# ioloizou/g1_locomotion

Hardware: AMD Instinct MI355X
Metric: QP solves/sec, SRBD N=10 12-state/12-input (higher is better)
Workload: dtype f64; 1 GPU; configs[1]: batch=4096/GPU random SRBD states, N=10, 2-contact alternating single support friction cone, fp64; tails deferred (SRBDQP_FLAG_DEFER_TAIL: the ~4 % of a batch that reach a rho-restart mark finish in the next launch on their stream; srbdqp_flush inside the timed region, every batch complete when the clock stops); steps rotate over 4 distinct device batches; horizon=10, batch_per_gpu=4096, kernel=wave_defer_f64_n10_s2, streams=2, longest_first_hint=False, deferred_tails=True, world_size=1, distinct_batches=4, max_iter=250, rho_restart_iter=0, rho_restart_count=0, set_up_dtype=f64

## Files before the change

### g1_locomotion_amd/csrc/srbdqp_common.hpp

```cpp
#pragma once
#include <cstddef>
#include <hip/hip_runtime.h>
#include <stdint.h>

namespace srbdqp {

constexpr int kThreads = 256;
constexpr double kInf = 1.0e30;

struct KArgs {
    const double* x0;
    const double* xref;
    const double* foot;
    const double* pcom;
    const double* warm_u;
    const double* warm_y;
    const uint8_t* contact;
    double* u_out;
    double* x_out;
    double* y_out;
    int32_t* status;
    int32_t* iters;
    double* P_out;
    double* q_out;
    double* l_out;
    double* ub_out;
    const int32_t* perm;
    int defer_x0;
    int tile_sel;
    const int32_t* row_off;
    long long* stamps;
    double* ws;
    const double* rho_qp;
    double* rho_out;
    const float* resid_in;
    float* resid_out;
    const int32_t* count_ptr;
    int32_t* cap_list;
    int32_t* cap_count;
    int32_t iters_base;
    int32_t restart_every;
    int32_t restart_max;
    int32_t inline_in;
    int32_t y_capped_only;
    int32_t qp_span;
    double* u_dev;
    char* tail_lists;
    int32_t* tail_cnt;
    int32_t tail_cap, tail_wgs, tail_iin, tail_iout, tail_izero;
    int32_t done_cs;
    int32_t* done_flag;
    int32_t* done_count;
    int32_t done_value;
    int32_t B;
    int32_t mode;
    int32_t max_iter, check_every;
    double dt, inv_mass, iinv[3], mu, fzmin_s, fzmax_s, s;
    double sqrtq[12];
    double rs2;
    double rho, rho_eq, sigma, alpha, eps_abs, eps_rel;
    double rho_fz;
};

template <int N>
struct StagedIn {
    double x0[13];
    double xref[13 * N];
    double foot[12 * N];
    double pcom[3 * N];
    uint8_t contact[4 * N];
    uint8_t pad[(8 - (4 * N) % 8) % 8];
};
template <int N>
__device__ __forceinline__ const char* staged_in_base(const KArgs& a) {
    static_assert(sizeof(KArgs) % 8 == 0, "StagedIn follows KArgs without padding");
    if constexpr (sizeof(KArgs) + sizeof(StagedIn<N>) > 4096) return nullptr;
    else return a.inline_in ? (const char*)__builtin_amdgcn_kernarg_segment_ptr() + sizeof(KArgs) : nullptr;
}

struct QpIo {
    const double *x0, *xref, *foot, *pcom;
    const uint8_t* contact;
    double *u_out, *x_out, *y_out;
    int32_t *status, *iters;
};
__device__ __forceinline__ QpIo io_of(const KArgs& a) { return QpIo{a.x0, a.xref, a.foot, a.pcom, a.contact, a.u_out, a.x_out, a.y_out, a.status, a.iters}; }
struct TailRecHead {
    int32_t b, pass, done, pad;
    double rho;
    QpIo io;
};
static_assert(sizeof(TailRecHead) <= 16 * sizeof(double), "the header of a tail record is 16 doubles");
constexpr int kTailRecDoubles = 16 + 3 * 64;
constexpr int kStatusPending = 0;

#define SRBDQP_QP_INDEX(a) ((a).perm ? (a).perm[blockIdx.x] : (int)blockIdx.x)

__device__ __forceinline__ double restart_rho_of(double rho0, const float* r) {
    const double num = (double)r[0] / fmax((double)r[1], 1e-30), den = (double)r[2] / fmax((double)r[3], 1e-30);
    double r1 = rho0;
    if (num > 0.0 && den > 0.0 && num <= 1.0e30 && den <= 1.0e30) r1 = fmin(fmax(rho0 * sqrt(num / den), rho0 * 0.1), rho0 * 5.0);
    return r1;
}
#define SRBDQP_RESTART_SKIP(a, b) ((a).resid_in && (a).status[(b)] != 2)
__device__ __forceinline__ double rho_of_qp(const KArgs& a, int b) {
    const double r0 = a.rho_qp ? a.rho_qp[b] : a.rho;
    const double r = a.resid_in ? restart_rho_of(r0, a.resid_in + (size_t)b * 4) : r0;
    if (a.rho_out && threadIdx.x == 0) a.rho_out[b] = r;
    return r;
}
#define SRBDQP_RHO_OF(a, b) rho_of_qp((a), (b))

__device__ __forceinline__ float uni(float v) { return __int_as_float(__builtin_amdgcn_readfirstlane(__float_as_int(v))); }
__device__ __forceinline__ double uni(double v) {
    const int lo = __builtin_amdgcn_readfirstlane(__double2loint(v)), hi = __builtin_amdgcn_readfirstlane(__double2hiint(v));
    return __hiloint2double(hi, lo);
}

__device__ __forceinline__ double unis(double v) {
    int lo, hi;
    asm volatile("s_nop 1\n\tv_readfirstlane_b32 %0, %2\n\tv_readfirstlane_b32 %1, %3" : "=s"(lo), "=s"(hi) : "v"(__double2loint(v)), "v"(__double2hiint(v)));
    return __hiloint2double(hi, lo);
}

constexpr int kAbStride = 18;
template <int N>
__device__ __forceinline__ void de_tables(const double* CP, const double* T1, const double* T2, const double* SQ, const double dt2, double* DE, const int t, const int nthreads, const int nl = N) {
    for (int it = t; it < 9 * N; it += nthreads) {
        const int m = it / 9, k = it - 9 * m, p = k / 3, q = k - 3 * p;
        const double* Cm = CP + 9 * m;
        const double* t1 = T1 + 9 * m;
        const double d4 = dt2 * dt2;
        const double e0 = SQ[0] * SQ[0] * t1[q], e1 = SQ[1] * SQ[1] * t1[3 + q], e2 = SQ[2] * SQ[2] * t1[6 + q];
        double v = T2[9 * m + k] + Cm[p] * e0 + Cm[3 + p] * e1 + Cm[6 + p] * e2;
        v *= d4;
        v += (p == q) ? (double)(nl - m) * dt2 * SQ[6 + p] * SQ[6 + p] : 0.0;
        DE[18 * m + k] = v;
        DE[18 * m + 9 + k] = d4 * ((p == 0) ? e0 : (p == 1) ? e1 : e2);
    }
}
template <int N>
__device__ __forceinline__ void kasm_rows(const double* Jb, const double* CP, const double* DE, const double* SQ, const uint8_t* act, const int n_eff, const double s,
                                          const double dt2m, const double dtm, double* AB, const int t, const int nthreads, const int nrows) {
    const double s2 = s * s, dt4m2 = dt2m * dt2m, dt2m2 = dtm * dtm;
    for (int r = t; r < nrows; r += nthreads) {
        const bool on = r < n_eff;
        const int rr = on ? r : 0;
        const int e = rr / 3, x = rr - 3 * e, gc = act[e], j = gc >> 2;
        const double* Jp = Jb + j * 36 + 3 * (gc & 3) + x;
        const double J0 = Jp[0], J1 = Jp[12], J2 = Jp[24];
        const double* C = CP + 9 * j;
        const double* D = DE + 18 * j;
        double v[16];
        v[0] = J0; v[1] = J1; v[2] = J2;
#pragma unroll
        for (int l = 0; l < 3; ++l) v[3 + l] = -(C[3 * l] * J0 + C[3 * l + 1] * J1 + C[3 * l + 2] * J2);
        v[6] = 1.0; v[7] = -(double)j;
#pragma unroll
        for (int l = 0; l < 6; ++l) v[8 + l] = s2 * (D[3 * l] * J0 + D[3 * l + 1] * J1 + D[3 * l + 2] * J2);
        const int Ls = N - j;
        const double al = (double)(((Ls - 1) * Ls * (2 * Ls - 1)) / 6), be = (double)(((Ls - 1) * Ls) / 2);
        const double fa = SQ[3 + x] * SQ[3 + x] * dt4m2, fb = SQ[9 + x] * SQ[9 + x] * dt2m2;
        v[14] = s2 * (fa * (al + (double)j * be) + fb * (double)Ls);
        v[15] = s2 * fa * be;
        typedef double d2 __attribute__((ext_vector_type(2)));
        d2* row = reinterpret_cast<d2*>(AB + kAbStride * r);
#pragma unroll
        for (int i = 0; i < 8; ++i) row[i] = on ? (d2){v[2 * i], v[2 * i + 1]} : (d2){0.0, 0.0};
    }
}

__device__ __forceinline__ void kasm_tile(const double* AB, const int ta, const int tb, const int mcol, const int kq, const int n_eff, const double dgxy, const double dgz,
                                          double (&out)[4]) {
    typedef double d2 __attribute__((ext_vector_type(2)));
    const int c = 16 * tb + mcol;
    double Bv[8];
    {
        const d2* row = reinterpret_cast<const d2*>(AB + kAbStride * c + 8);
#pragma unroll
        for (int i = 0; i < 4; ++i) { const d2 v = row[i]; Bv[2 * i] = v[0]; Bv[2 * i + 1] = v[1]; }
    }
    const int cm3 = c - 3 * ((c * 0xAAAB) >> 17);
    const double dcol = (c < n_eff) ? ((cm3 < 2) ? dgxy : dgz) : 1.0;
#pragma unroll
    for (int q = 0; q < 4; ++q) {
        const int r = 16 * ta + kq + 4 * q;
        const d2* row = reinterpret_cast<const d2*>(AB + kAbStride * r);
        double Av[8];
#pragma unroll
        for (int i = 0; i < 4; ++i) { const d2 v = row[i]; Av[2 * i] = v[0]; Av[2 * i + 1] = v[1]; }
        double v = Av[0] * Bv[0];
#pragma unroll
        for (int i = 1; i < 6; ++i) v = fma(Av[i], Bv[i], v);
        const double ft = fma(Av[7], Bv[7], Av[6] * Bv[6]);
        const int d = r + 3 * 1024 - c, dm3 = d - 3 * ((d * 0xAAAB) >> 17);
        v += (dm3 == 0) ? ft : 0.0;
        v += (r == c) ? dcol : 0.0;
        out[q] = v;
    }
}

template <int N>
__device__ __forceinline__ double gx_row(const double* CP, const double* TF, const int i, const int kk, const double dt, const double dt2, const double dtm, const double dt2m) {
    double acc = 0.0;
    if (kk < 3) {
        const double* Ci = CP + i * 9 + kk * 3;
        const double c0 = Ci[0], c1 = Ci[1], c2 = Ci[2];
#pragma unroll 4
        for (int j = 0; j < N; ++j) {
            const double* Cj = CP + j * 9 + kk * 3;
            const double* tau = TF + 6 * j;
            const double term = (c0 - Cj[0]) * tau[0] + (c1 - Cj[1]) * tau[1] + (c2 - Cj[2]) * tau[2];
            acc += (j <= i) ? term : 0.0;
        }
        return acc * dt2;
    } else if (kk < 6) {
#pragma unroll 4
        for (int j = 0; j < N; ++j) { const double v = TF[6 * j + kk]; acc += (j <= i) ? (double)(i - j) * v : 0.0; }
        return acc * dt2m;
    } else {
#pragma unroll 4
        for (int j = 0; j < N; ++j) { const double v = TF[6 * j + kk - 6]; acc += (j <= i) ? v : 0.0; }
        return acc * ((kk < 9) ? dt : dtm);
    }
}

constexpr int kFirstCheck = 0;

#define SRBDQP_STAMP(a, b, idx) do { if ((a).stamps && threadIdx.x == 0) (a).stamps[(size_t)(b) * 16 + (idx)] = (long long)__builtin_amdgcn_s_memtime(); } while (0)

__device__ __forceinline__ void signal_done(const KArgs& a) {
    if (!a.done_flag) return;
    __threadfence_system();
    __syncthreads();
    if (threadIdx.x == 0) {
        bool last = true;
        if (a.B > 1) {
            last = (atomicAdd(a.done_count, 1) == a.B - 1);
            if (last) *a.done_count = 0;
        }
        if (last) __hip_atomic_store(a.done_flag, a.done_value, __ATOMIC_RELAXED, __HIP_MEMORY_SCOPE_SYSTEM);
    }
}

__device__ __forceinline__ unsigned long long done_cs_pack(int status, int iters) { return (unsigned long long)(unsigned)status | ((unsigned long long)(unsigned)iters << 32); }
__device__ __forceinline__ unsigned dpp_xor_row(unsigned v) {
    v ^= (unsigned)__builtin_amdgcn_update_dpp((int)v, (int)v, 0xB1, 0xF, 0xF, false);
    v ^= (unsigned)__builtin_amdgcn_update_dpp((int)v, (int)v, 0x4E, 0xF, 0xF, false);
    v ^= (unsigned)__builtin_amdgcn_update_dpp((int)v, (int)v, 0x141, 0xF, 0xF, false);
    v ^= (unsigned)__builtin_amdgcn_update_dpp((int)v, (int)v, 0x140, 0xF, 0xF, false);
    return v;
}
template <int BT>
__device__ __forceinline__ void signal_done_checksum(int32_t* done_flag, int32_t done_value, unsigned long long cs) {
    static_assert(BT % 16 == 0 && BT / 16 <= 16, "one 16-byte record per row of 16 lanes in 256 bytes");
    const unsigned lo = dpp_xor_row((unsigned)cs), hi = dpp_xor_row((unsigned)(cs >> 32));
    if ((threadIdx.x & 15) == 0) {
        uint4 v;
        v.x = (unsigned)done_value; v.y = (unsigned)(BT / 16); v.z = lo; v.w = hi;
        reinterpret_cast<uint4*>(done_flag)[threadIdx.x >> 4] = v;
    }
}

template <int N>
struct Dims {
    static constexpr int n = 12 * N;
    static constexpr int m = 20 * N;
    static constexpr int gtot = 72 * N * (N + 1);
    static constexpr int ME = (m + kThreads - 1) / kThreads;
    static constexpr int VE = (n + kThreads - 1) / kThreads;
};

template <int N, class L>
__device__ void load_and_linearise(const KArgs& a, int b, double* sm) {
    using S = L;
    const int t = threadIdx.x;
    const char* kin_ = staged_in_base<N>(a);
    const double* gx0 = kin_ ? reinterpret_cast<const double*>(kin_ + offsetof(StagedIn<N>, x0)) : a.x0 + (size_t)b * 13;
    const double* gxr = kin_ ? reinterpret_cast<const double*>(kin_ + offsetof(StagedIn<N>, xref)) : a.xref + (size_t)b * N * 13;
    const double* gft = kin_ ? reinterpret_cast<const double*>(kin_ + offsetof(StagedIn<N>, foot)) : a.foot + (size_t)b * N * 12;
    const uint8_t* gct = kin_ ? reinterpret_cast<const uint8_t*>(kin_ + offsetof(StagedIn<N>, contact)) : a.contact + (size_t)b * N * 4;
    uint8_t* sct = reinterpret_cast<uint8_t*>(sm + S::o_ct);
    constexpr int RX = (N * 13 + kThreads - 1) / kThreads, RF = (N * 12 + kThreads - 1) / kThreads;
    static_assert(N * 4 <= kThreads, "one thread per contact flag");
    const double* gpc = a.pcom ? (kin_ ? reinterpret_cast<const double*>(kin_ + offsetof(StagedIn<N>, pcom)) : a.pcom + (size_t)b * N * 3) : gx0;
    const double v_x0 = gx0[t < 13 ? t : 0];
    const uint8_t v_ct = gct[t < N * 4 ? t : 0];
    const double v_pc = gpc[(a.pcom && t < N * 3) ? t : 0];
    double v_xr[RX], v_ft[RF];
#pragma unroll
    for (int r = 0; r < RX; ++r) { const int i = t + r * kThreads; v_xr[r] = gxr[i < N * 13 ? i : 0]; }
#pragma unroll
    for (int r = 0; r < RF; ++r) { const int i = t + r * kThreads; v_ft[r] = gft[i < N * 12 ? i : 0]; }
    if (t < 13) sm[S::o_x0 + t] = v_x0;
    if (t >= 32 && t < 44) sm[S::o_sq + t - 32] = a.sqrtq[t - 32];
#pragma unroll
    for (int r = 0; r < RX; ++r) { const int i = t + r * kThreads; if (i < N * 13) sm[S::o_xref + i] = v_xr[r]; }
#pragma unroll
    for (int r = 0; r < RF; ++r) { const int i = t + r * kThreads; if (i < N * 12) sm[S::o_foot + i] = v_ft[r]; }
    if (t < N * 4) sct[t] = v_ct ? 1 : 0;
    if (a.pcom && t < N * 3) sm[S::o_pcom + t] = v_pc;
    __syncthreads();
    if (!a.pcom && t < N * 3) sm[S::o_pcom + t] = sm[S::o_xref + (t / 3) * 13 + 3 + (t % 3)];
    if (t < N) {
        double sn, cs;
        sincos(sm[S::o_xref + t * 13 + 2], &sn, &cs);
        double* T = sm + S::o_tm + t * 9;
        T[0] = cs;  T[1] = sn;  T[2] = 0.0;
        T[3] = -sn; T[4] = cs;  T[5] = 0.0;
        T[6] = 0.0; T[7] = 0.0; T[8] = 1.0;
    }
    __syncthreads();
    if (t < 9) {
        double acc = 0.0;
        for (int k = 0; k < N; ++k) { acc += sm[S::o_tm + k * 9 + t]; sm[S::o_cp + k * 9 + t] = acc; }
    }
    if (t < N * 12) {
        const int k = t / 12, cc = t % 12, ci = cc / 3, ax = cc % 3;
        const double cs = sm[S::o_tm + k * 9 + 0], sn = sm[S::o_tm + k * 9 + 1];
        const double i0 = a.iinv[0], i1 = a.iinv[1], i2 = a.iinv[2];
        const double w00 = cs * cs * i0 + sn * sn * i1, w01 = cs * sn * (i0 - i1), w11 = sn * sn * i0 + cs * cs * i1;
        const double rx = sm[S::o_foot + k * 12 + 3 * ci + 0] - sm[S::o_pcom + k * 3 + 0];
        const double ry = sm[S::o_foot + k * 12 + 3 * ci + 1] - sm[S::o_pcom + k * 3 + 1];
        const double rz = sm[S::o_foot + k * 12 + 3 * ci + 2] - sm[S::o_pcom + k * 3 + 2];
        const double s0 = (ax == 0) ? 0.0 : ((ax == 1) ? -rz : ry);
        const double s1 = (ax == 0) ? rz : ((ax == 1) ? 0.0 : -rx);
        const double s2 = (ax == 0) ? -ry : ((ax == 1) ? rx : 0.0);
        double* J = sm + S::o_J + k * 36;
        J[0 * 12 + cc] = w00 * s0 + w01 * s1;
        J[1 * 12 + cc] = w01 * s0 + w11 * s1;
        J[2 * 12 + cc] = i2 * s2;
    }
    __syncthreads();
}

template <int N, class L>
__device__ __forceinline__ double free_response(const KArgs& a, const double* sm, int i, int kk) {
    using S = L;
    const double* x0 = sm + S::o_x0;
    if (kk < 3) {
        const double* C = sm + S::o_cp + i * 9 + kk * 3;
        return x0[kk] + a.dt * (C[0] * x0[6] + C[1] * x0[7] + C[2] * x0[8]);
    } else if (kk < 6) {
        double v = x0[kk] + (double)(i + 1) * a.dt * x0[kk + 6];
        if (kk == 5) v += a.dt * a.dt * x0[12] * (double)((i * (i + 1)) / 2);
        return v;
    } else if (kk < 9) {
        return x0[kk];
    } else {
        double v = x0[kk];
        if (kk == 11) v += (double)(i + 1) * a.dt * x0[12];
        return v;
    }
}

template <int N, class L>
__device__ __forceinline__ void eh_entry(const KArgs& a, double* sm, const double* SQ, const int k) {
    const int i = k / 12, kk = k - 12 * i;
    sm[L::o_eh + k] = SQ[kk] * (free_response<N, L>(a, sm, i, kk) - sm[L::o_xref + i * 13 + kk]);
}

template <int N, class L>
__device__ __forceinline__ double free_response_sel(const KArgs& a, const double* sm, int i, int kk) {
    const double* x0 = sm + L::o_x0;
    const double* C = sm + L::o_cp + i * 9 + (kk < 3 ? kk : 0) * 3;
    const double xk = x0[kk];
    const double vr = xk + a.dt * (C[0] * x0[6] + C[1] * x0[7] + C[2] * x0[8]);
    const double vp = xk + (double)(i + 1) * a.dt * x0[(kk >= 3 && kk < 6) ? kk + 6 : 6];
    const double vz = vp + a.dt * a.dt * x0[12] * (double)((i * (i + 1)) / 2);
    const double vw = xk + (double)(i + 1) * a.dt * x0[12];
    return (kk < 3) ? vr : (kk < 5) ? vp : (kk == 5) ? vz : (kk == 11) ? vw : xk;
}

template <int N>
__device__ __forceinline__ void de_step(const double (&Cm)[9], const double (&t1)[9], const double (&t2)[9], const double* SQ, const double dt2, const int m, double* de) {
    const double d4 = dt2 * dt2;
#pragma unroll
    for (int k = 0; k < 9; ++k) {
        const int p = k / 3, q = k - 3 * p;
        const double e0 = SQ[0] * SQ[0] * t1[q], e1 = SQ[1] * SQ[1] * t1[3 + q], e2 = SQ[2] * SQ[2] * t1[6 + q];
        double v = t2[k] + Cm[p] * e0 + Cm[3 + p] * e1 + Cm[6 + p] * e2;
        v *= d4;
        if (p == q) v += (double)(N - m) * dt2 * SQ[6 + p] * SQ[6 + p];
        de[k] = v;
        de[9 + k] = d4 * ((p == 0) ? e0 : (p == 1) ? e1 : e2);
    }
}

__device__ __forceinline__ double lane_bcast(double v, int l) {
    const int lo = __builtin_amdgcn_readlane(__double2loint(v), l), hi = __builtin_amdgcn_readlane(__double2hiint(v), l);
    return __hiloint2double(hi, lo);
}

template <int NV>
__device__ __forceinline__ void block_max(double (&v)[NV], double* red) {
    const int lane = threadIdx.x & 63, wave = threadIdx.x >> 6;
#pragma unroll
    for (int q = 0; q < NV; ++q) {
        double x = v[q];
#pragma unroll
        for (int off = 32; off >= 1; off >>= 1) x = fmax(x, __shfl_xor(x, off));
        if (lane == 0) red[wave * 8 + q] = x;
    }
    __syncthreads();
#pragma unroll
    for (int q = 0; q < NV; ++q) v[q] = fmax(fmax(red[q], red[8 + q]), fmax(red[16 + q], red[24 + q]));
    __syncthreads();
}

template <int N, class L, int BT = kThreads, bool CS = false>
__device__ void rollout_and_store_to(const KArgs& a, double* u_out, double* x_out, int b, double* sm, const double* uh, double* scratch , unsigned long long* cs = nullptr) {
    using S = L;
    constexpr int n = Dims<N>::n;
    const int t = threadIdx.x;
    for (int c = t; c < n; c += BT) {
        const double v = a.s * uh[c];
        u_out[(size_t)b * n + c] = v;
        if constexpr (CS) *cs ^= (unsigned long long)__double_as_longlong(v);
    }
    if (a.u_dev) for (int c = t; c < n; c += BT) a.u_dev[(size_t)b * n + c] = a.s * uh[c];
    if (!x_out) return;
    const double* x0 = sm + S::o_x0;
    double* sj = scratch + 6 * N;
    for (int idx = t; idx < 6 * N; idx += BT) {
        const int j = idx / 6, comp = idx % 6;
        const double* u = uh + 12 * j;
        double s;
        if (comp < 3) {
            const double* J = sm + S::o_J + j * 36 + comp * 12;
            s = 0.0;
            for (int c = 0; c < 12; ++c) s += J[c] * u[c];
            if (__ballot(!(fabs(s) <= kInf)) != 0ull) {
                s = 0.0;
                for (int c = 0; c < 12; ++c) s = (u[c] != 0.0) ? fma(J[c], u[c], s) : s;
            }
        } else {
            const int ax = comp - 3;
            s = (u[ax] + u[3 + ax] + u[6 + ax] + u[9 + ax]) * a.inv_mass;
        }
        sj[idx] = s;
    }
    __syncthreads();
    for (int idx = t; idx < 6 * N; idx += BT) {
        const int k = idx / 6 + 1, comp = idx % 6;
        double acc = 0.0;
        if constexpr (N <= 12) {
#pragma unroll
            for (int j = 0; j < N; ++j) { const double sv = sj[6 * j + comp]; acc += (j < k) ? sv : 0.0; }
        } else {
            for (int j = 0; j < k; ++j) acc += sj[6 * j + comp];
        }
        double v = x0[6 + comp] + a.dt * a.s * acc;
        if (comp == 5) v += (double)k * a.dt * x0[12];
        scratch[idx] = v;
    }
    __syncthreads();
    double* pa = sj;
    constexpr int PA_OFF = (64 * ((3 * N + 63) / 64) + 3 * N <= BT) ? 64 * ((3 * N + 63) / 64) : 3 * N;
    for (int tt = t; tt < PA_OFF + 3 * N; tt += BT) {
        if (tt < 3 * N || tt >= PA_OFF) {
            const bool posn = tt >= PA_OFF;
            const int e = posn ? tt - PA_OFF : tt;
            const int k = e / 3 + 1, comp = e % 3 + (posn ? 3 : 0);
            double acc;
            if (posn) {
                acc = x0[6 + comp];
                if constexpr (N <= 12) {
#pragma unroll
                    for (int l = 1; l < N; ++l) { const double sv = scratch[(l - 1) * 6 + comp]; acc += (l < k) ? sv : 0.0; }
                } else {
                    for (int l = 1; l < k; ++l) acc += scratch[(l - 1) * 6 + comp];
                }
            } else {
                acc = 0.0;
                auto term_of = [&](int l) {
                    const double* T = sm + S::o_tm + l * 9 + comp * 3;
                    const double* w = (l == 0) ? (x0 + 6) : (scratch + (l - 1) * 6);
                    return T[0] * w[0] + T[1] * w[1] + T[2] * w[2];
                };
                if constexpr (N <= 12) {
#pragma unroll
                    for (int l = 0; l < N; ++l) { const double term = term_of(l); acc += (l < k) ? term : 0.0; }
                } else {
                    for (int l = 0; l < k; ++l) acc += term_of(l);
                }
            }
            pa[6 * (k - 1) + comp] = x0[comp] + a.dt * acc;
        }
    }
    __syncthreads();
    double* xo = x_out + (size_t)b * (N + 1) * 13;
    for (int idx = t; idx < 13 * (N + 1); idx += BT) {
        const int k = idx / 13, comp = idx % 13;
        const double* src = (k == 0 || comp == 12) ? (x0 + comp) : ((comp >= 6) ? (scratch + (k - 1) * 6 + comp - 6) : (pa + (k - 1) * 6 + comp));
        const double v = *src;
        xo[idx] = v;
        if constexpr (CS) *cs ^= (unsigned long long)__double_as_longlong(v);
    }
}
template <int N, class L, int BT = kThreads>
__device__ __forceinline__ void rollout_and_store(const KArgs& a, int b, double* sm, const double* uh, double* scratch ) {
    rollout_and_store_to<N, L, BT>(a, a.u_out, a.x_out, b, sm, uh, scratch);
}

}
```

### g1_locomotion_amd/csrc/srbdqp_setup1.hpp

```cpp
#pragma once
#include "srbdqp_split.hpp"

namespace srbdqp {

#ifdef SRBDQP_WAVE_STAMPS
#define WSTAMP(a, b, idx) SRBDQP_STAMP(a, b, idx)
#define WSTAMP_RT(a, b, idx) do { if ((a).stamps && threadIdx.x == 0) (a).stamps[(size_t)(b) * 16 + (idx)] = (long long)__builtin_amdgcn_s_memrealtime(); } while (0)
#else
#define WSTAMP(a, b, idx) do { } while (0)
#define WSTAMP_RT(a, b, idx) do { } while (0)
#endif

template <int N, int MAXS>
struct Setup1Smem {
    using S = CompactSmem<N, MAXS>;
    static constexpr int n = Dims<N>::n;
    static constexpr int up2(int v) { return (v + 1) & ~1; }
    static constexpr int o_x0 = S::o_x0, o_tm = S::o_tm, o_J = S::o_J;
    static constexpr int o_cp = S::o_R;
    static constexpr int o_mt = o_cp + up2(9 * N);
    static constexpr int o_ab = o_mt + 18 * N;
    static constexpr int o_gv = o_mt + up2(9 * S::NPAIR);
    static constexpr int o_t1 = o_gv + up2(9 * N);
    static constexpr int o_t2 = o_t1 + up2(9 * N);
    static constexpr int o_x0c = o_t1;
    static constexpr int o_tf = o_x0c + up2(S::nmax) + 16;
    static constexpr int endT = (o_t2 + up2(9 * N) > o_tf + 6 * N) ? o_t2 + up2(9 * N) : o_tf + 6 * N;
    static constexpr int o_xref = up2(endT);
    static constexpr int o_foot = o_xref + up2(N * 13);
    static constexpr int o_pcom = o_foot + N * 12;
    static constexpr int o_eh = o_foot;
    static constexpr int o_gx = o_foot;
    static constexpr int o_scr = o_xref;
    static constexpr int endIn = o_pcom + up2(N * 3);
    static constexpr int endIn2 = (endIn > o_scr + 258) ? endIn : o_scr + 258;
    static constexpr int kStgRow = 18;
    static constexpr int kStgTile = 16 * kStgRow;
    static constexpr int endStg = (endIn2 > o_cp + S::NT * kStgTile) ? endIn2 : o_cp + S::NT * kStgTile;
    static constexpr int endAb = o_ab + 16 * S::NT * kAbStride;
    static constexpr int o_end = endStg > endAb ? endStg : endAb;
    static constexpr size_t bytes = (size_t)o_end * sizeof(double);
    static constexpr bool supported = SplitWs<N, MAXS>::supported && S::NT <= 4;
    static_assert(n + 6 * N <= o_end - o_eh || true, "");
};

template <int N, int MAXS, bool FUSED, bool DUMP, bool PHI, int RP>
__device__ __forceinline__ bool setup1_pass(const KArgs& a, const QpIo& io, const int b, double* sm, double& rho_b, int& rs_pass, int& rs_done) {
    using S = CompactSmem<N, MAXS>;
    using W = SplitWs<N, MAXS>;
    using L1 = Setup1Smem<N, MAXS>;
    constexpr int n = Dims<N>::n, m = Dims<N>::m, NT = S::NT;
    int lane = threadIdx.x;
    if constexpr (RP == 2) asm volatile("" : "+v"(lane));
    [[maybe_unused]] double* const park = sm + L1::o_end;
    int mcol = lane & 15, kq = lane >> 4;
    double* ws = FUSED ? nullptr : a.ws + (size_t)b * W::doubles;
    int* icnt = reinterpret_cast<int*>(sm + S::o_int);
    int* imisc = icnt + 2 * N;
    uint8_t* act = reinterpret_cast<uint8_t*>(imisc + 8);
    uint8_t* sct = reinterpret_cast<uint8_t*>(sm + S::o_ct);
    const double* SQ = sm + S::o_sq;
    const double* CP = sm + L1::o_cp;

    WSTAMP(a, b, 0);
    WSTAMP_RT(a, b, 12);
    constexpr int JT = (12 * N + 63) / 64;
    double yc, ys;
    [[maybe_unused]] double v_xr[JT];
    if constexpr (RP == 2) {
        const int k = lane < N ? lane : 0;
        yc = sm[S::o_tm + k * 9 + 0];
        ys = sm[S::o_tm + k * 9 + 1];
    } else {
        const double* gx0 = io.x0 + (size_t)b * 13;
        const double* gxr = io.xref + (size_t)b * N * 13;
        const double* gft = io.foot + (size_t)b * N * 12;
        const uint8_t* gct = io.contact + (size_t)b * N * 4;
        const double* gpc = io.pcom ? io.pcom + (size_t)b * N * 3 : nullptr;
        const double v_x0 = gx0[lane < 13 ? lane : 0];
        const uint8_t v_ct = gct[lane < 4 * N ? lane : 0];
        const double v_yaw = gxr[(lane < N ? lane : 0) * 13 + 2];
        double v_f[JT][3], v_p[JT][3];
#pragma unroll
        for (int t = 0; t < JT; ++t) {
            const int tt = (lane + 64 * t < 12 * N) ? lane + 64 * t : 0;
            const int k = tt / 12, ci = (tt % 12) / 3;
            const double* pc = gpc ? gpc + k * 3 : gxr + k * 13 + 3;
#pragma unroll
            for (int c = 0; c < 3; ++c) { v_f[t][c] = gft[k * 12 + 3 * ci + c]; v_p[t][c] = pc[c]; }
            v_xr[t] = gxr[k * 13 + (tt - 12 * k)];
        }
        sincos(v_yaw, &ys, &yc);
        if (lane < 13) sm[S::o_x0 + lane] = v_x0;
        if (lane >= 32 && lane < 44) sm[S::o_sq + lane - 32] = a.sqrtq[lane - 32];
        if (lane < N * 4) sct[lane] = v_ct ? 1 : 0;
        if (lane < N) {
            double* T = sm + S::o_tm + lane * 9;
            T[0] = yc;  T[1] = ys;  T[2] = 0.0;
            T[3] = -ys; T[4] = yc;  T[5] = 0.0;
            T[6] = 0.0; T[7] = 0.0; T[8] = 1.0;
        }
        {
            const bool flag = (lane < 4 * N) && v_ct != 0;
            const unsigned long long bal = __ballot(flag);
            if (flag) act[__popcll(bal & ((1ull << lane) - 1ull))] = (uint8_t)lane;
            if (lane < N) icnt[lane] = __popcll(bal & ((4 * (lane + 1) >= 64) ? ~0ull : ((1ull << (4 * (lane + 1))) - 1ull)));
            const bool over = lane < N && __popcll((bal >> (4 * (lane < N ? lane : 0))) & 0xFull) > MAXS;
            const unsigned long long viol = __ballot(over);
            if (lane == 0) {
                imisc[0] = __popcll(bal);
                imisc[1] = viol != 0ull;
                sm[S::o_misc] = 0.0;
                sm[S::o_misc + 1] = 0.0;
            }
        }
#pragma unroll
        for (int t = 0; t < JT; ++t) {
            const int tt = lane + 64 * t;
            const int k = (tt < 12 * N ? tt : 0) / 12, cc = tt - 12 * k, ax = cc % 3;
            const double cs = __shfl(yc, k), sn = __shfl(ys, k);
            const double i0 = a.iinv[0], i1 = a.iinv[1], i2 = a.iinv[2];
            const double w00 = cs * cs * i0 + sn * sn * i1, w01 = cs * sn * (i0 - i1), w11 = sn * sn * i0 + cs * cs * i1;
            const double rx = v_f[t][0] - v_p[t][0];
            const double ry = v_f[t][1] - v_p[t][1];
            const double rz = v_f[t][2] - v_p[t][2];
            const double s0 = (ax == 0) ? 0.0 : ((ax == 1) ? -rz : ry);
            const double s1 = (ax == 0) ? rz : ((ax == 1) ? 0.0 : -rx);
            const double s2 = (ax == 0) ? -ry : ((ax == 1) ? rx : 0.0);
            if (tt < 12 * N) {
                double* J = sm + S::o_J + k * 36;
                J[0 * 12 + cc] = w00 * s0 + w01 * s1;
                J[1 * 12 + cc] = w01 * s0 + w11 * s1;
                J[2 * 12 + cc] = i2 * s2;
            }
        }
    }
    double ccu[N], csu[N], ccm = 0.0, csm = 0.0;
    {
        double ac = 0.0, as = 0.0;
#pragma unroll
        for (int k = 0; k < N; ++k) {
            const double c = lane_bcast(yc, k), s = lane_bcast(ys, k);
            ac += c;
            as += s;
            ccu[k] = ac;
            csu[k] = as;
            ccm += (k <= lane) ? c : 0.0;
            csm += (k <= lane) ? s : 0.0;
        }
    }
    if (lane < N) {
        double* C = sm + L1::o_cp + lane * 9;
        C[0] = ccm;  C[1] = csm; C[2] = 0.0;
        C[3] = -csm; C[4] = ccm; C[5] = 0.0;
        C[6] = 0.0;  C[7] = 0.0; C[8] = (double)(lane + 1);
    }
    __syncthreads();
    const int na = imisc[0];
    const int n_eff = 3 * na;
    double* xs0 = sm + L1::o_mt;
    static_assert(L1::o_end - L1::o_mt >= n + 12 * N, "early-exit scratch");
    if (RP != 2 && (imisc[1] != 0 || na == 0)) {
        if constexpr (DUMP) { if (lane == 0) a.ub_out[(size_t)b * m] = (imisc[1] != 0) ? -1.0 : 0.0; return false; }
        for (int c = lane; c < n; c += 64) xs0[c] = 0.0;
        if (io.y_out) for (int i = lane; i < m; i += 64) io.y_out[(size_t)b * m + i] = 0.0;
        if (lane == 0) {
            if (io.status) io.status[b] = (imisc[1] != 0) ? kStatusContactBound : 1;
            if (io.iters) io.iters[b] = a.iters_base;
            if constexpr (!FUSED) ws[S::o_misc + 1] = 1.0;
        }
        __syncthreads();
        rollout_and_store_to<N, S, 64>(a, io.u_out, io.x_out, b, sm, xs0, xs0 + n);
        return false;
    }

    WSTAMP(a, b, 1);
    const double dt = a.dt, dt2 = a.dt * a.dt, dtm = a.dt * a.inv_mass, dt2m = dt2 * a.inv_mass;
    double* DE = sm + L1::o_mt;
    double* GV = sm + L1::o_gv;
    if constexpr (RP != 2) {
#pragma unroll
        for (int t = 0; t < JT; ++t) {
            const int k = lane + 64 * t;
            const int kc = k < n ? k : 0, i = kc / 12, kk = kc - 12 * i;
            const double v = SQ[kk] * (free_response_sel<N, L1>(a, sm, i, kk) - v_xr[t]);
            if (k < n) sm[L1::o_eh + k] = v;
        }
    }
    if (lane < N) {
        const int mm = lane;
        const double w0 = SQ[0] * SQ[0], w1 = SQ[1] * SQ[1], w2 = SQ[2] * SQ[2];
        double t1a = 0.0, t1b = 0.0, t2aa = 0.0, t2ab = 0.0, t2bb = 0.0, t2zz = 0.0;
#pragma unroll
        for (int i = 0; i < N; ++i) {
            const bool on = i >= mm;
            const double da = ccu[i] - ccm, db = csu[i] - csm, dz = (double)(i - mm);
            t1a += on ? da : 0.0;
            t1b += on ? db : 0.0;
            t2aa += on ? (w0 * da) * da + (w1 * db) * db : 0.0;
            t2ab += on ? (w0 * da) * db - (w1 * db) * da : 0.0;
            t2bb += on ? (w0 * db) * db + (w1 * da) * da : 0.0;
            t2zz += on ? (w2 * dz) * dz : 0.0;
        }
        const double t1z = (double)(((N - mm) * (N - mm - 1)) / 2);
        const double Cm[9] = {ccm, csm, 0.0, -csm, ccm, 0.0, 0.0, 0.0, (double)(mm + 1)};
        const double t1[9] = {t1a, t1b, 0.0, -t1b, t1a, 0.0, 0.0, 0.0, t1z};
        const double t2[9] = {t2aa, t2ab, 0.0, t2ab, t2bb, 0.0, 0.0, 0.0, t2zz};
        de_step<N>(Cm, t1, t2, SQ, dt2, mm, DE + 18 * mm);
    }
    auto gt_tables = [&](const double* vec) {
        for (int e = lane; e < 3 * N; e += 64) {
            const int j = e / 3, comp = e - 3 * j;
            const double* Cj = CP + j * 9;
            double acc = 0.0;
#pragma unroll
            for (int i = 0; i < N; ++i) {
                const double* Ci = CP + i * 9;
                const double* v = vec + 12 * i;
                const double term = dt2 * ((Ci[comp] - Cj[comp]) * (SQ[0] * v[0]) + (Ci[3 + comp] - Cj[3 + comp]) * (SQ[1] * v[1]) +
                                           (Ci[6 + comp] - Cj[6 + comp]) * (SQ[2] * v[2])) + dt * (SQ[6 + comp] * v[6 + comp]);
                acc += (i >= j) ? term : 0.0;
            }
            GV[9 * j + comp] = acc;
        }
        constexpr int HL = (3 * N) % 64;
        for (int e = lane - HL; e < 6 * N; e += 64) {
            if (e < 0) continue;
            const int j = e / 6, comp = 3 + (e - 6 * j);
            double acc = 0.0;
            const int off = (comp < 6) ? comp : 3 + comp;
#pragma unroll
            for (int i = 0; i < N; ++i) {
                const double v = vec[12 * i + off];
                const double term = (comp < 6) ? (double)(i - j) * v : v;
                acc += (i >= j) ? term : 0.0;
            }
            GV[9 * j + comp] = acc;
        }
    };
    auto gt_eval = [&](int c) -> double {
        const int e = c / 3, ax = c - 3 * e, gc = act[e], j = gc >> 2;
        const double* J = sm + S::o_J + j * 36 + 3 * (gc & 3) + ax;
        const double* g = GV + 9 * j;
        return a.s * (J[0] * g[0] + J[12] * g[1] + J[24] * g[2] + SQ[3 + ax] * dt2m * g[3 + ax] + SQ[9 + ax] * dtm * g[6 + ax]);
    };
    __syncthreads();
    if constexpr (RP != 2) gt_tables(sm + L1::o_eh);
    __syncthreads();
    WSTAMP(a, b, 2);
    if constexpr (RP != 2) for (int c = lane; c < n_eff; c += 64) sm[S::o_q + c] = gt_eval(c);
    if (RP >= 2 || a.warm_u) {
        double* TF = sm + L1::o_tf;
        for (int c = lane; c < n_eff; c += 64)
            sm[L1::o_x0c + c] = (RP >= 2 ? park[c] : a.warm_u[(size_t)b * n + 3 * act[c / 3] + (c % 3)]) / a.s;
        __syncthreads();
        for (int tt = lane; tt < 6 * N; tt += 64) {
            const int j = tt / 6, comp = tt - 6 * j;
            double acc = 0.0;
            for (int e = (j ? icnt[j - 1] : 0); e < icnt[j]; ++e) {
                const double* x = sm + L1::o_x0c + 3 * e;
                if (comp < 3) {
                    const double* J = sm + S::o_J + j * 36 + comp * 12 + 3 * (act[e] & 3);
                    acc += J[0] * x[0] + J[1] * x[1] + J[2] * x[2];
                } else {
                    acc += x[comp - 3];
                }
            }
            TF[tt] = acc;
        }
        __syncthreads();
        for (int k = lane; k < n; k += 64) {
            const int i = k / 12, kk = k - 12 * i;
            const double acc = gx_row<N>(CP, TF, i, kk, dt, dt2, dtm, dt2m);
            sm[L1::o_gx + k] = SQ[kk] * a.s * acc;
        }
        __syncthreads();
        gt_tables(sm + L1::o_gx);
        __syncthreads();
        for (int c = lane; c < n_eff; c += 64) sm[S::o_px0 + c] = gt_eval(c) + a.rs2 * sm[L1::o_x0c + c];
    } else {
        for (int c = lane; c < n_eff; c += 64) sm[S::o_px0 + c] = 0.0;
    }

    if constexpr (PHI) {
        double* phi = ws + W::o_phi;
        const double x0_keep = (lane < 13) ? sm[S::o_x0 + lane] : 0.0;
        for (int kc = 0; kc < 13; ++kc) {
            __syncthreads();
            if (lane < 13) sm[S::o_x0 + lane] = (lane == kc) ? 1.0 : 0.0;
            __syncthreads();
            for (int k = lane; k < n; k += 64) {
                const int i = k / 12, kk = k - 12 * i;
                sm[L1::o_eh + k] = SQ[kk] * free_response<N, L1>(a, sm, i, kk);
            }
            __syncthreads();
            gt_tables(sm + L1::o_eh);
            __syncthreads();
            for (int c = lane; c < n_eff; c += 64) phi[c * 13 + kc] = gt_eval(c);
        }
        __syncthreads();
        if (lane < 13) sm[S::o_x0 + lane] = x0_keep;
        __syncthreads();
    }
    WSTAMP(a, b, 3);
    v4d Kt[NT][NT];
    __syncthreads();
    {
        double* AB = sm + L1::o_ab;
        kasm_rows<N>(sm + S::o_J, CP, DE, SQ, act, n_eff, a.s, dt2m, dtm, AB, lane, 64, 16 * NT);
        __syncthreads();
        typedef double d2 __attribute__((ext_vector_type(2)));
        const double dgxy = uni(a.rs2 + a.sigma + 2.0 * rho_b), dgz = uni(a.rs2 + a.sigma + (4.0 * a.mu * a.mu + a.rho_fz) * rho_b);
        const int d3 = (mcol - kq + 3) % 3;
        const double ind[3] = {d3 == 0 ? 1.0 : 0.0, d3 == 1 ? 1.0 : 0.0, d3 == 2 ? 1.0 : 0.0};
        double eqd[4];
#pragma unroll
        for (int q = 0; q < 4; ++q) eqd[q] = (kq + 4 * q == mcol) ? 1.0 : 0.0;
        double Bv[NT][8], dcol[NT];
#pragma unroll
        for (int tb = 0; tb < NT; ++tb) {
            const int c = 16 * tb + mcol;
            const d2* row = reinterpret_cast<const d2*>(AB + kAbStride * c + 8);
#pragma unroll
            for (int i = 0; i < 4; ++i) { const d2 v = row[i]; Bv[tb][2 * i] = v[0]; Bv[tb][2 * i + 1] = v[1]; }
            dcol[tb] = (c < n_eff) ? (((tb + mcol) % 3 < 2) ? dgxy : dgz) : 1.0;
        }
#pragma unroll
        for (int ta = 0; ta < NT; ++ta) {
#pragma unroll
            for (int q = 0; q < 4; ++q) {
                const int r = 16 * ta + kq + 4 * q;
                const d2* row = reinterpret_cast<const d2*>(AB + kAbStride * r);
                double Av[8];
#pragma unroll
                for (int i = 0; i < 4; ++i) { const d2 v = row[i]; Av[2 * i] = v[0]; Av[2 * i + 1] = v[1]; }
#pragma unroll
                for (int tb = ta; tb < NT; ++tb) {
                    double v = Av[0] * Bv[tb][0];
#pragma unroll
                    for (int i = 1; i < 6; ++i) v = fma(Av[i], Bv[tb][i], v);
                    const double ft = fma(Av[7], Bv[tb][7], Av[6] * Bv[tb][6]);
                    v = fma(ind[((ta + q - tb) % 3 + 3) % 3], ft, v);
                    if (ta == tb) v = fma(eqd[q], dcol[tb], v);
                    Kt[ta][tb][q] = v;
                }
            }
        }
    }
    __syncthreads();
    WSTAMP(a, b, 4);
    WSTAMP(a, b, 5);
    if constexpr (DUMP) {
        dump_presolved<N>(a, b, n_eff, na, sm + S::o_q, act, [&](auto&& put) {
#pragma unroll
            for (int ta = 0; ta < NT; ++ta)
#pragma unroll
                for (int tb = ta; tb < NT; ++tb)
#pragma unroll
                    for (int q = 0; q < 4; ++q)
                        if (16 * ta + kq + 4 * q <= 16 * tb + mcol) put(16 * ta + kq + 4 * q, 16 * tb + mcol, Kt[ta][tb][q]);
        });
        return false;
    }

    double* scr = sm + L1::o_scr;
    auto a_operand_read = [&](double (&op)[4]) {
#pragma unroll
        for (int r = 0; r < 4; ++r) op[r] = scr[mcol * 16 + ((4 * r + kq) ^ mcol)];
        asm volatile("" ::: "memory");
    };
    auto a_operand = [&](const v4d& x, double (&op)[4]) {
        asm volatile("" ::: "memory");
#pragma unroll
        for (int q = 0; q < 4; ++q) {
            const int row = kq + 4 * q;
            scr[row * 16 + (mcol ^ row)] = x[q];
        }
        asm volatile("" ::: "memory");
        a_operand_read(op);
    };
    const v4d zero4 = (v4d){0.0, 0.0, 0.0, 0.0};

    bool all_ok = true;
#pragma unroll
    for (int j = 0; j < NT; ++j) {
        bool ok;
        const v4d w = diag16_invert_dpp_packed(Kt[j][j], lane, ok, scr);
        all_ok = all_ok && ok;
        Kt[j][j] = w;
        if (j + 1 < NT) {
            double wa[4];
            a_operand_read(wa);
#pragma unroll
            for (int bb = j + 1; bb < NT; ++bb) {
                v4d o = zero4;
#pragma unroll
                for (int r = 0; r < 4; ++r) o = mfma_f64(wa[r], Kt[j][bb][r], o);
                Kt[j][bb] = o;
            }
#pragma unroll
            for (int aa = j + 1; aa < NT; ++aa)
#pragma unroll
                for (int bb = aa; bb < NT; ++bb)
#pragma unroll
                    for (int r = 0; r < 4; ++r) Kt[aa][bb] = mfma_f64(-Kt[j][aa][r], Kt[j][bb][r], Kt[aa][bb]);
        }
    }
    if (!all_ok && lane == 0) sm[S::o_misc] = 1.0;
    WSTAMP(a, b, 6);

#pragma unroll
    for (int i = 1; i < NT; ++i) {
        double wa[4];
        a_operand(Kt[i][i], wa);
#pragma unroll
        for (int j = 0; j < i; ++j) {
            v4d sacc = zero4;
#pragma unroll
            for (int k = j; k < i; ++k) {
                const v4d& wkj = (k == j) ? Kt[j][j] : Kt[j][k];
#pragma unroll
                for (int r = 0; r < 4; ++r) sacc = mfma_f64(Kt[k][i][r], wkj[r], sacc);
            }
            v4d o = zero4;
#pragma unroll
            for (int r = 0; r < 4; ++r) o = mfma_f64(-wa[r], sacc[r], o);
            Kt[j][i] = o;
        }
    }

    WSTAMP(a, b, 7);
    double kin[W::KS];
    if constexpr (!FUSED) {
        for (int i = lane; i < S::o_R; i += 64) ws[i] = sm[i];
        double* kinv = ws + W::o_kinv;
#pragma unroll
        for (int aa = 0; aa < NT; ++aa) {
#pragma unroll
            for (int bb = aa; bb < NT; ++bb) {
                v4d o = zero4;
#pragma unroll
                for (int k = bb; k < NT; ++k) {
                    const v4d& wka = (k == aa) ? Kt[aa][aa] : Kt[aa][k];
                    const v4d& wkb = (k == bb) ? Kt[bb][bb] : Kt[bb][k];
#pragma unroll
                    for (int r = 0; r < 4; ++r) o = mfma_f64(wka[r], wkb[r], o);
                }
                const int col = 16 * bb + mcol;
#pragma unroll
                for (int q = 0; q < 4; ++q) {
                    const int row = 16 * aa + kq + 4 * q;
                    if (row < n_eff && col < W::KS) kinv[row * W::KS + col] = (col < n_eff) ? o[q] : 0.0;
                    if (aa != bb && col < n_eff && row < W::KS) kinv[col * W::KS + row] = (row < n_eff) ? o[q] : 0.0;
                }
            }
        }
    } else {
        double* stg = sm + L1::o_cp;
        static_assert(L1::o_end - L1::o_cp >= NT * L1::kStgTile, "staging of one block column of K^-1");
        const int grp = lane >> 4;
        v4d Ku[NT][NT];
#pragma unroll
        for (int cb = NT - 1; cb >= 0; --cb) {
            asm volatile("" ::: "memory");
#pragma unroll
            for (int g = 0; g <= cb; ++g) {
                v4d o = zero4;
#pragma unroll
                for (int k = cb; k < NT; ++k) {
                    const v4d& wkg = (k == g) ? Kt[g][g] : Kt[g][k];
                    const v4d& wkc = (k == cb) ? Kt[cb][cb] : Kt[cb][k];
#pragma unroll
                    for (int r = 0; r < 4; ++r) o = mfma_f64(wkg[r], wkc[r], o);
                }
#pragma unroll
                for (int q = 0; q < 4; ++q) stg[g * L1::kStgTile + (kq + 4 * q) * L1::kStgRow + mcol] = o[q];
                if (g < cb) Ku[g][cb] = o;
            }
#pragma unroll
            for (int g = cb + 1; g < NT; ++g)
#pragma unroll
                for (int q = 0; q < 4; ++q) stg[g * L1::kStgTile + mcol * L1::kStgRow + kq + 4 * q] = Ku[cb][g][q];
            asm volatile("" ::: "memory");
            const double2* rowp = reinterpret_cast<const double2*>(stg + grp * L1::kStgTile + mcol * L1::kStgRow);
#pragma unroll
            for (int h = 0; h < 8; ++h) {
                if (16 * cb + 2 * h + 1 < W::KS + 1) {
                    const double2 v = rowp[h];
                    if (16 * cb + 2 * h < W::KS) kin[16 * cb + 2 * h] = v.x;
                    if (16 * cb + 2 * h + 1 < W::KS) kin[16 * cb + 2 * h + 1] = v.y;
                }
            }
            asm volatile("" ::: "memory");
        }
    }
    if constexpr (FUSED) {
        if (__builtin_amdgcn_readfirstlane(n_eff) < W::KS) {
#pragma unroll
            for (int c = 0; c < W::KS; ++c) kin[c] = (lane < n_eff && c < n_eff) ? kin[c] : 0.0;
        }
        __syncthreads();
        WSTAMP(a, b, 8);
        WSTAMP(a, b, 9);
        static_assert(L1::o_end >= SplitSmem<N, MAXS>::o_end, "the ADMM body's vectors live in this kernel's LDS");
        if constexpr (RP == 0) {
            admm_wave_body<N, MAXS>(a, b, rho_b, sm, kin);
        } else {
            WaveRestart rs;
            const int left = a.max_iter - rs_done;
            rs.pass = rs_pass;
            rs.more = rs_pass < a.restart_max && a.restart_every < left;
            rs.kcap = rs.more ? a.restart_every : left;
            rs.park = park;
            int status = -1, iters = 0;
            admm_wave_iterations<N, MAXS, true>(a, io, RP == 1 ? a.warm_u : nullptr, RP == 1 ? a.warm_y : nullptr, b, rho_b, sm, kin, sm + SplitSmem<N, MAXS>::o_xs,
                                                status, iters, &rs);
            rs_done += iters;
            if (status == 2 && rs.more) {
                rho_b = restart_rho_of(rho_b, rs.v);
                ++rs_pass;
                __syncthreads();
                return true;
            }
            admm_wave_finish<N, MAXS>(a, io, b, sm, status, rs_done);
        }
        WSTAMP(a, b, 10);
        WSTAMP(a, b, 11);
        WSTAMP_RT(a, b, 13);
    }
    return false;
}

template <int N, int MAXS, bool FUSED, bool DUMP = false, bool PHI = false, bool RST = false>
__global__ __launch_bounds__(64, 2) void srbdqp_setup1_kernel(KArgs a) {
    static_assert(!(PHI && FUSED), "dq/dx0 is a hand-over of the split pipeline");
    static_assert(!RST || (FUSED && !DUMP), "the restart in place belongs to the fused solve");
    static_assert(Setup1Smem<N, MAXS>::supported, "one wave holds all tiles: at most 4 x 4 tiles");
    static_assert(4 * N <= 64, "one ballot compacts the contact flags");
    extern __shared__ __attribute__((aligned(16))) double sm[];
    if ((int)blockIdx.x >= a.B) return;
    if (a.count_ptr && (int)blockIdx.x >= *a.count_ptr) return;
    const int b = SRBDQP_QP_INDEX(a);
    if (SRBDQP_RESTART_SKIP(a, b)) return;
    double rho_b = SRBDQP_RHO_OF(a, b);
    int rs_pass = 0, rs_done = 0;
    const QpIo io = io_of(a);
    if constexpr (!RST) {
        setup1_pass<N, MAXS, FUSED, DUMP, PHI, 0>(a, io, b, sm, rho_b, rs_pass, rs_done);
    } else {
        bool again = setup1_pass<N, MAXS, FUSED, DUMP, PHI, 1>(a, io, b, sm, rho_b, rs_pass, rs_done);
        if (!again) return;
        again = setup1_pass<N, MAXS, FUSED, DUMP, PHI, 2>(a, io, b, sm, rho_b, rs_pass, rs_done);
        if (!again) return;
        again = setup1_pass<N, MAXS, FUSED, DUMP, PHI, 2>(a, io, b, sm, rho_b, rs_pass, rs_done);
        if (!again) return;
        KArgs al = a;
        al.restart_max = 0;
        setup1_pass<N, MAXS, FUSED, DUMP, PHI, 2>(al, io, b, sm, rho_b, rs_pass, rs_done);
    }
}

__device__ __forceinline__ unsigned long long unis_u64(unsigned long long v) {
    int lo, hi;
    asm volatile("s_nop 1\n\tv_readfirstlane_b32 %0, %2\n\tv_readfirstlane_b32 %1, %3" : "=s"(lo), "=s"(hi) : "v"((int)(unsigned)v), "v"((int)(unsigned)(v >> 32)));
    return ((unsigned long long)(unsigned)hi << 32) | (unsigned long long)(unsigned)lo;
}
template <typename T> __device__ __forceinline__ T* unis_ptr(T* p) { return reinterpret_cast<T*>(unis_u64(reinterpret_cast<unsigned long long>(p))); }

__device__ __forceinline__ double* tail_claim(const KArgs& a) {
    int slot = 0;
    if (threadIdx.x == 0) slot = atomicAdd(a.tail_cnt + a.tail_iout, 1);
    slot = __builtin_amdgcn_readfirstlane(slot);
    if (slot >= a.tail_cap) return nullptr;
    return reinterpret_cast<double*>(a.tail_lists) + ((size_t)a.tail_iout * (size_t)a.tail_cap + (size_t)slot) * kTailRecDoubles;
}

__device__ __forceinline__ bool tail_export(const KArgs& a, const QpIo& io, int b, double rho_b, int rs_pass, int rs_done, const double* park) {
    const int lane = threadIdx.x;
    double* rec = tail_claim(a);
    if (!rec) return false;
    if (lane == 0) {
        TailRecHead* hd = reinterpret_cast<TailRecHead*>(rec);
        hd->b = b; hd->pass = rs_pass; hd->done = rs_done; hd->pad = 0; hd->rho = rho_b; hd->io = io;
        if (io.status) io.status[b] = kStatusPending;
    }
    rec[16 + lane] = park[lane]; rec[80 + lane] = park[64 + lane]; rec[144 + lane] = park[128 + lane];
    return true;
}

template <int N, int MAXS, bool FLUSH = false>
__global__ __launch_bounds__(64, 2) void srbdqp_wave_defer_kernel(KArgs a) {
    static_assert(Setup1Smem<N, MAXS>::supported && 4 * N <= 64, "the one-wave kernel's limits");
    extern __shared__ __attribute__((aligned(16))) double sm[];
    using L1 = Setup1Smem<N, MAXS>;
    const int lane = threadIdx.x;
    const int T = a.tail_wgs;
    double* const park = sm + L1::o_end;
    auto in_place = [&](const QpIo& io, const int b, double rho_b, int rs_pass, int rs_done) __attribute__((always_inline)) {
        bool again = setup1_pass<N, MAXS, true, false, false, 2>(a, io, b, sm, rho_b, rs_pass, rs_done);
        if (!again) return;
        again = setup1_pass<N, MAXS, true, false, false, 2>(a, io, b, sm, rho_b, rs_pass, rs_done);
        if (!again) return;
        KArgs al = a;
        al.restart_max = 0;
        setup1_pass<N, MAXS, true, false, false, 2>(al, io, b, sm, rho_b, rs_pass, rs_done);
    };
    if ((int)blockIdx.x < T) {
        const int i = blockIdx.x;
        int cnt = a.tail_cnt[a.tail_iin];
        cnt = cnt < a.tail_cap ? cnt : a.tail_cap;
        if (i == 0 && lane == 0) a.tail_cnt[a.tail_izero] = 0;
        const double* lin = reinterpret_cast<const double*>(a.tail_lists) + (size_t)a.tail_iin * (size_t)a.tail_cap * kTailRecDoubles;
        if (i >= cnt) return;
        const double* rec = lin + (size_t)i * kTailRecDoubles;
        const TailRecHead* hd = reinterpret_cast<const TailRecHead*>(rec);
        QpIo io;
        io.x0 = unis_ptr(hd->io.x0); io.xref = unis_ptr(hd->io.xref); io.foot = unis_ptr(hd->io.foot); io.pcom = unis_ptr(hd->io.pcom);
        io.contact = unis_ptr(hd->io.contact); io.u_out = unis_ptr(hd->io.u_out); io.x_out = unis_ptr(hd->io.x_out); io.y_out = unis_ptr(hd->io.y_out);
        io.status = unis_ptr(hd->io.status); io.iters = unis_ptr(hd->io.iters);
        const int b = __builtin_amdgcn_readfirstlane(hd->b);
        int rs_pass = __builtin_amdgcn_readfirstlane(hd->pass), rs_done = __builtin_amdgcn_readfirstlane(hd->done);
        double rho_b = unis(hd->rho);
        park[lane] = rec[16 + lane]; park[64 + lane] = rec[80 + lane]; park[128 + lane] = rec[144 + lane];
        __syncthreads();
        if (!setup1_pass<N, MAXS, true, false, false, 3>(a, io, b, sm, rho_b, rs_pass, rs_done)) return;
        if constexpr (!FLUSH) { if (tail_export(a, io, b, rho_b, rs_pass, rs_done, park)) return; }
        in_place(io, b, rho_b, rs_pass, rs_done);
    } else if constexpr (!FLUSH) {
        const int wg = (int)blockIdx.x - T;
        if (wg >= a.B) return;
        const int b = a.perm ? a.perm[wg] : wg;
        double rho_b = a.rho_qp ? a.rho_qp[b] : a.rho;
        int rs_pass = 0, rs_done = 0;
        const QpIo io = io_of(a);
        if (!setup1_pass<N, MAXS, true, false, false, 1>(a, io, b, sm, rho_b, rs_pass, rs_done)) return;
        if (tail_export(a, io, b, rho_b, rs_pass, rs_done, park)) return;
        in_place(io, b, rho_b, rs_pass, rs_done);
    }
}

}
```

Before: 40.25 million QP/s.

## Precompute per step-pair terms into LDS for setup triangular sums

Replaces the per-lane O(N) triangular accumulation in the setup (prefix cosine/sine sums and the weighted quadratic terms) with a lane-per-step-pair precompute stored in LDS. Each lane then sums only its triangle slice from the shared table. The G'v tables get the same treatment, and de_step folds its diagonal term into FMAs. The goal is less redundant per-lane arithmetic and register pressure (the ccu/csu arrays are dropped), at the cost of extra LDS traffic, barriers and changed floating-point rounding order.

```diff
diff --git a/g1_locomotion_amd/csrc/srbdqp_common.hpp b/g1_locomotion_amd/csrc/srbdqp_common.hpp
--- a/g1_locomotion_amd/csrc/srbdqp_common.hpp
+++ b/g1_locomotion_amd/csrc/srbdqp_common.hpp
@@ -380,8 +380,12 @@
         const int p = k / 3, q = k - 3 * p;
         const double e0 = SQ[0] * SQ[0] * t1[q], e1 = SQ[1] * SQ[1] * t1[3 + q], e2 = SQ[2] * SQ[2] * t1[6 + q];
         double v = t2[k] + Cm[p] * e0 + Cm[3 + p] * e1 + Cm[6 + p] * e2;
-        v *= d4;
-        if (p == q) v += (double)(N - m) * dt2 * SQ[6 + p] * SQ[6 + p];
+        if (p == q) {
+            const double x = (double)(N - m) * dt2 * SQ[6 + p];
+            v = (p < 2) ? fma(SQ[6 + p], x, d4 * v) : fma(d4, v, SQ[6 + p] * x);
+        } else {
+            v *= d4;
+        }
         de[k] = v;
         de[9 + k] = d4 * ((p == 0) ? e0 : (p == 1) ? e1 : e2);
     }
diff --git a/g1_locomotion_amd/csrc/srbdqp_setup1.hpp b/g1_locomotion_amd/csrc/srbdqp_setup1.hpp
--- a/g1_locomotion_amd/csrc/srbdqp_setup1.hpp
+++ b/g1_locomotion_amd/csrc/srbdqp_setup1.hpp
@@ -40,7 +40,13 @@
     static constexpr int endAb = o_ab + 16 * S::NT * kAbStride;
     static constexpr int o_end = endStg > endAb ? endStg : endAb;
     static constexpr size_t bytes = (size_t)o_end * sizeof(double);
+    static constexpr int kPairs = S::NPAIR;
+    static constexpr int kPairSlots = (N / 2) * N + N;
+    static constexpr int o_pd = o_t1;
+    static constexpr int o_pq = up2(endIn);
+    static constexpr bool pairs_fit = N % 2 == 0 && kPairs <= 64 && 2 * kPairSlots <= 2 * up2(9 * N) && o_pq + 4 * kPairSlots <= o_end;
     static constexpr bool supported = SplitWs<N, MAXS>::supported && S::NT <= 4;
+    static_assert(!supported || pairs_fit, "a lane and an LDS slot for every step pair of a horizon the one-wave kernel takes");
     static_assert(n + 6 * N <= o_end - o_eh || true, "");
 };
 
@@ -135,19 +141,12 @@
             }
         }
     }
-    double ccu[N], csu[N], ccm = 0.0, csm = 0.0;
-    {
-        double ac = 0.0, as = 0.0;
-#pragma unroll
-        for (int k = 0; k < N; ++k) {
-            const double c = lane_bcast(yc, k), s = lane_bcast(ys, k);
-            ac += c;
-            as += s;
-            ccu[k] = ac;
-            csu[k] = as;
-            ccm += (k <= lane) ? c : 0.0;
-            csm += (k <= lane) ? s : 0.0;
-        }
+    double ccm = 0.0, csm = 0.0;
+#pragma unroll
+    for (int k = 0; k < N; ++k) {
+        const double c = lane_bcast(yc, k), s = lane_bcast(ys, k);
+        ccm += (k <= lane) ? c : 0.0;
+        csm += (k <= lane) ? s : 0.0;
     }
     if (lane < N) {
         double* C = sm + L1::o_cp + lane * 9;
@@ -187,21 +186,45 @@
             if (k < n) sm[L1::o_eh + k] = v;
         }
     }
+    const int pair_c = lane < L1::kPairs ? lane : L1::kPairs - 1;
+    const int pair_r = pair_c / (N + 1), pair_k = pair_c - pair_r * (N + 1);
+    const bool pair_lo = pair_k < N - pair_r;
+    const int pair_m = pair_lo ? pair_r : N - 1 - pair_r, pair_i = pair_m + (pair_lo ? pair_k : pair_k - (N - pair_r));
+    const double pair_da = CP[9 * pair_i] - CP[9 * pair_m], pair_db = CP[9 * pair_i + 1] - CP[9 * pair_m + 1];
+    double* PD = sm + L1::o_pd;
+    double* PQ = sm + L1::o_pq;
+    {
+        const double w0 = SQ[0] * SQ[0], w1 = SQ[1] * SQ[1], w2 = SQ[2] * SQ[2];
+        const double da = pair_da, db = pair_db, dz = (double)(pair_i - pair_m);
+        if (lane < L1::kPairs) {
+            PD[2 * lane] = da;
+            PD[2 * lane + 1] = db;
+            PQ[4 * lane] = fma(w0 * da, da, (w1 * db) * db);
+            PQ[4 * lane + 1] = fma(w0 * da, db, -((w1 * db) * da));
+            PQ[4 * lane + 2] = fma(w0 * db, db, (w1 * da) * da);
+            PQ[4 * lane + 3] = (pair_i == N - 1) ? 0.0 : (w2 * dz) * dz;
+        }
+    }
+    __syncthreads();
+    const int pair_base = (2 * lane < N) ? lane * (N + 1) : (N - lane) * N;
     if (lane < N) {
         const int mm = lane;
-        const double w0 = SQ[0] * SQ[0], w1 = SQ[1] * SQ[1], w2 = SQ[2] * SQ[2];
         double t1a = 0.0, t1b = 0.0, t2aa = 0.0, t2ab = 0.0, t2bb = 0.0, t2zz = 0.0;
 #pragma unroll
-        for (int i = 0; i < N; ++i) {
-            const bool on = i >= mm;
-            const double da = ccu[i] - ccm, db = csu[i] - csm, dz = (double)(i - mm);
-            t1a += on ? da : 0.0;
-            t1b += on ? db : 0.0;
-            t2aa += on ? (w0 * da) * da + (w1 * db) * db : 0.0;
-            t2ab += on ? (w0 * da) * db - (w1 * db) * da : 0.0;
-            t2bb += on ? (w0 * db) * db + (w1 * da) * da : 0.0;
-            t2zz += on ? (w2 * dz) * dz : 0.0;
-        }
+        for (int s = 0; s < N; ++s) {
+            if (s < N - mm) {
+                const double* pd = PD + 2 * (pair_base + s);
+                const double* pq = PQ + 4 * (pair_base + s);
+                t1a += pd[0];
+                t1b += pd[1];
+                t2aa += pq[0];
+                t2ab += pq[1];
+                t2bb += pq[2];
+                t2zz += pq[3];
+            }
+        }
+        const double dzl = (double)(N - 1 - mm);
+        t2zz = fma((SQ[2] * SQ[2]) * dzl, dzl, t2zz);
         const double t1z = (double)(((N - mm) * (N - mm - 1)) / 2);
         const double Cm[9] = {ccm, csm, 0.0, -csm, ccm, 0.0, 0.0, 0.0, (double)(mm + 1)};
         const double t1[9] = {t1a, t1b, 0.0, -t1b, t1a, 0.0, 0.0, 0.0, t1z};
@@ -209,31 +232,39 @@
         de_step<N>(Cm, t1, t2, SQ, dt2, mm, DE + 18 * mm);
     }
     auto gt_tables = [&](const double* vec) {
-        for (int e = lane; e < 3 * N; e += 64) {
-            const int j = e / 3, comp = e - 3 * j;
-            const double* Cj = CP + j * 9;
+        {
+            const double* v = vec + 12 * pair_i;
+            const double p0 = SQ[0] * v[0], p1 = SQ[1] * v[1], p2 = SQ[2] * v[2], dz = (double)(pair_i - pair_m);
+            if (lane < L1::kPairs) {
+                PQ[4 * lane] = fma(dt, SQ[6] * v[6], dt2 * fma(pair_da, p0, (-pair_db) * p1));
+                PQ[4 * lane + 1] = fma(dt, SQ[7] * v[7], dt2 * fma(pair_db, p0, pair_da * p1));
+                PQ[4 * lane + 2] = fma(dt, SQ[8] * v[8], dt2 * (dz * p2));
+            }
+        }
+        __syncthreads();
+        if (lane < 3 * N) {
+            const int j = lane / 3, comp = lane - 3 * j;
+            const double* pq = PQ + 4 * ((2 * j < N) ? j * (N + 1) : (N - j) * N) + comp;
             double acc = 0.0;
 #pragma unroll
-            for (int i = 0; i < N; ++i) {
-                const double* Ci = CP + i * 9;
-                const double* v = vec + 12 * i;
-                const double term = dt2 * ((Ci[comp] - Cj[comp]) * (SQ[0] * v[0]) + (Ci[3 + comp] - Cj[3 + comp]) * (SQ[1] * v[1]) +
-                                           (Ci[6 + comp] - Cj[6 + comp]) * (SQ[2] * v[2])) + dt * (SQ[6 + comp] * v[6 + comp]);
-                acc += (i >= j) ? term : 0.0;
-            }
+            for (int s = 0; s < N; ++s)
+                if (s < N - j) acc += pq[4 * s];
             GV[9 * j + comp] = acc;
         }
-        constexpr int HL = (3 * N) % 64;
-        for (int e = lane - HL; e < 6 * N; e += 64) {
-            if (e < 0) continue;
-            const int j = e / 6, comp = 3 + (e - 6 * j);
-            double acc = 0.0;
-            const int off = (comp < 6) ? comp : 3 + comp;
-#pragma unroll
-            for (int i = 0; i < N; ++i) {
-                const double v = vec[12 * i + off];
-                const double term = (comp < 6) ? (double)(i - j) * v : v;
-                acc += (i >= j) ? term : 0.0;
+        static_assert(6 * N <= 64, "the force entries of the G'v tables are one trip of the wave");
+        if (lane < 6 * N) {
+            const int j = lane / 6, comp = 3 + (lane - 6 * j);
+            const double* v = vec + 12 * j + ((comp < 6) ? comp : 3 + comp);
+            const double winc = (comp < 6) ? 1.0 : 0.0;
+            double acc = 0.0, w = (comp < 6) ? 0.0 : 1.0;
+#pragma unroll
+            for (int s = 0; s < N; ++s) {
+                if (s < N - j) {
+                    double term = w * v[12 * s];
+                    asm volatile("" : "+v"(term));
+                    acc += term;
+                }
+                w += winc;
             }
             GV[9 * j + comp] = acc;
         }
```

New measurement: 40.85 million QP/s, median of 6. +1.5%, better.
